# Kitware/SMQTK-Indexing

Measured on AMD Instinct MI355X. Metric: queries/sec, exact brute-force l2 kNN k=100 over 10000000x128 float32 (recall@100 = 1.0 by construction); scan HBM GB/s vs 8 TB/s peak, higher is better.
Workload: dtype f32 results (distances bit-identical to numpy float32); filter arithmetic int8 MFMA (i32 accumulation, measured per-row error bound), exact re-rank f32

## Files before the change

### smqtk_indexing_amd/csrc/sq_dense.hip

```cpp
#include <algorithm>
#include <type_traits>
#include <vector>
#include <cmath>

#include "sq_dense_exact.hpp"
#include "sq_dense_scan.hpp"
#include "sq_dense_mid.hpp"
#include "sq_dense_i8.hpp"
#include "sq_dense_wide.hpp"
#include "sq_dense_i8_wide.hpp"
#include "sq_dense_tighten.hpp"
#include "sq_dense_remove.hpp"

namespace sq {

struct DenseCall {
    bool pending = false;
    const float* q = nullptr;
    int nq = 0, k = 0, nq_pad = 0;
    void* out_dist = nullptr;
    long long* out_idx = nullptr;
    hipStream_t st = nullptr;
    bool small = false, all_fallback = false, prof = false, use_event = false, int8 = false;
    bool mid_direct = false;
// ... 560 lines not shown
            hipGraph_t g = nullptr;
            bool ok = hipStreamBeginCapture(st, hipStreamCaptureModeThreadLocal) == hipSuccess;
            if (ok) {
                const int rc = chain(st, static_cast<const DenseCallPtrs*>(ind_dev));
                const hipError_t ec = hipStreamEndCapture(st, &g);
                ok = rc == SQ_OK && ec == hipSuccess && g != nullptr;
            }
            if (ok) ok = hipGraphInstantiate(&s.gexec, g, nullptr, nullptr, 0) == hipSuccess;
            if (g) (void)hipGraphDestroy(g);
            if (!ok) {
                (void)hipGetLastError();
                s.gexec = nullptr;
                h->graph_broken = true;
            } else {
                s.gkey = key;
                if (getenv("SQ_INT8_REPORT")) fprintf(stderr, "[smqtk_hip] call graph captured (%d queries, k = %d)\n", c.nq, c.k);
            }
        }
        s.seen_key = key;
        if (s.gexec) {
            *static_cast<DenseCallPtrs*>(s.call_ptrs.p) = DenseCallPtrs{c.q, c.out_dist, c.out_idx};
            SQ_HIP(hipGraphLaunch(s.gexec, st));
            return SQ_OK;
        }
    }
    return chain(st, nullptr);
}

static int dense8_enqueue(DenseHandle* h, DenseSlot& s, const DenseCtx& e) {
    const long long n = h->n;
    DenseCall& c = s.call;
    const int d = h->d;
    c.int8 = true;
    dense8_rearm(h);
    const int row8 = h->row8, unit_rows = i8_unit_rows(row8), spu = 2 * (unit_rows / 32), waves8 = i8_waves(row8);
    const long long n_units = (n + unit_rows - 1) / unit_rows;
    long long stride = h->opt.sample_stride;
    if (stride <= 0) {
        stride = (long long)((row8 == 128 ? 14.0 : 10.0) * sqrt((double)n / 1e7 * 100.0 / (double)e.kk / (double)e.qt) / (e.cosine ? 1.9 : 1.0) + 0.5);
        if (stride > 16) stride = 16;
        const bool will_tighten = h->opt.dense_fused != 0 && h->opt.dense_tighten != 0 && e.qt == 1 && e.nqt == 1;
        if (will_tighten) {
            stride = (long long)(40.0 * sqrt((double)n / 1e7 * 100.0 / (double)e.kk) + 0.5);
            if (stride > 64) stride = 64;
        }
        if (stride < 1) stride = 1;
        if (stride > (long long)e.cap / (16ll * e.kk)) stride = std::max<long long>(1, (long long)e.cap / (16ll * e.kk));
    }
    while (stride > 1 && (n_units / stride) * spu < 8ll * e.kk) stride >>= 1;
    const long long ns_units = (n_units + stride - 1) / stride;
    const long long ns = ns_units * spu;
    SQ_TRY(s.keys.reserve((size_t)c.nq * e.key_stride * e.key_bytes));
    SQ_TRY(s.q8.reserve((size_t)2 * c.nq_pad * row8));
    SQ_TRY(s.par8.reserve((size_t)c.nq_pad * 8));
    const int cus = cu_count(h->device);
    int nrb_sample = 0;
    const int nrb = dense_pass_blocks(h->opt, c.use_event, e.nqt, cus, 0, nrb_sample);
    const long long n_waves = (long long)nrb * e.nqt * waves8;
    const int ldq = (d + 3) / 4 * 4;
    SQ_TRY(s.wave_out.reserve((size_t)n_waves * kWaveCap * 8));
    SQ_TRY(s.wave_cnt.reserve((size_t)n_waves * 8));
    SQ_TRY(s.q_al.reserve((size_t)c.nq * ldq * 4));
    const float* centerp = (!e.cosine && h->center.p) ? h->center.as<float>() : nullptr;
    Dense8ScanArgs a{};
    a.scan8 = h->scan8.as<signed char>();
    a.nrow = h->nrow8.as<float>();
    a.n = n;
    a.n_units = n_units;
    a.qs8 = s.q8.as<signed char>();
    a.par = s.par8.as<float2>();
    a.thr = e.thr;
    a.wave_out = s.wave_out.as<uint2>();
    a.wave_cnt = s.wave_cnt.as<u32>();
    a.wave_cap = kWaveCap;
    a.sample_out = s.sample.as<float>();
    a.ns = ns;
    a.nqt = e.nqt;
    a.plane_rows = c.nq_pad;
    a.debug = h->opt.dense_debug;
    dense_nt_policy(h->opt, (size_t)h->n_pad64 * row8, row8, 64, e.nqt == 1, a.nt, a.nt_from_row);
    if (ns_units < (long long)nrb_sample * waves8) nrb_sample = (int)(((ns_units + waves8 - 1) / waves8 + 7) / 8 * 8);
    bool fused = h->opt.dense_fused != 0 && e.qt == 1 && e.nqt == 1 && ns_units >= 2ll * e.kk;
    const bool tighten = fused && h->opt.dense_tighten != 0;
    if (fused) {
        const int lanes_per_wg = waves8 * 2;
        const int wg_min = ((4 * e.kk + lanes_per_wg - 1) / lanes_per_wg + 7) / 8 * 8, wg_max = 2048 / lanes_per_wg;
        if (wg_min > wg_max || wg_min > cus)
            fused = false;
        else
            nrb_sample = std::min(std::max(nrb_sample, wg_min), std::min(wg_max, (cus + 7) / 8 * 8));
    }
    int keep8 = waves8 * 2;
    if (fused) {
        const double per_wg = (double)e.kk / nrb_sample;
        if (per_wg <= 1.7 && keep8 > 4) keep8 = 4;
        else if (per_wg <= 4.5 && keep8 > 8) keep8 = 8;
    }
    const long long lane_m = (long long)nrb_sample * keep8;
    SQ_TRY(s.sample.reserve(fused ? (size_t)TILE_ROWS * lane_m * 4 : (size_t)c.nq_pad * ns * 4));
    a.sample_out = s.sample.as<float>();
    if (fused) {
        SQ_TRY(s.wave_score.reserve((size_t)n_waves * kWaveCap * 4));
        SQ_TRY(s.hist8.reserve((size_t)I8_HIST_WORDS * 4));
        a.wave_score = s.wave_score.as<float>();
        a.hist = s.hist8.as<u32>();
    }
    int wpb = 2;
    if (!e.cosine && h->opt.dense_rerank_segments > 0 && waves8 % h->opt.dense_rerank_segments == 0 && h->opt.dense_rerank_segments <= 4)
        wpb = h->opt.dense_rerank_segments;
    const double* cnx = h->cos_nx.as<double>();
    auto chain = [&](hipStream_t cs, const DenseCallPtrs* ind) -> int {
        if (fused) {
            Dense8HeadArgs ha{};
            ha.s = a;
            ha.s.unit_step = stride;
            ha.s.n_sel = ns_units;
            ha.s.nrb = nrb_sample;
            ha.q = c.q;
            ha.nq = c.nq;
            ha.d = d;
            ha.center = centerp;
            ha.dx = h->dx8;
            ha.r_max = h->rmax8;
            ha.x_max = h->xmax8;
            ha.cosine = e.cosine ? 1 : 0;
            ha.qn2 = e.qn2;
            ha.cnt = e.cnt;
            ha.oflag = e.oflag;
            ha.q_al = s.q_al.as<float>();
            ha.ldq = ldq;
            ha.ind = ind;
            ha.lane_min = s.sample.as<float>();
            ha.keep = keep8;
            ha.kk = e.kk;
            SQ_TRY(dense8_head_launch(row8, ha, cs));
            Dense8ScanArgs b = a;
            b.unit_step = 1;
            b.n_sel = n_units;
            b.nrb = nrb;
            Dense8TailArgs ta{h->db, h->ld, d, s.q_al.as<float>(), ldq, c.nq, s.keys.p, e.cnt, e.cap, e.oflag, cnx, e.cnq, h->opt.dense_debug, e.qn2, e.kk,
                              tighten ? 1 : 0, nullptr};
            s.clk8_wgs = 0;
            if ((h->opt.dense_debug & 8192) && !c.use_event) {
                SQ_TRY(s.clk8.reserve((size_t)nrb * 64));
                SQ_HIP(hipMemsetAsync(s.clk8.p, 0, (size_t)nrb * 64, cs));
                ta.clk = s.clk8.as<long long>();
                s.clk8_wgs = nrb;
            }
            if (c.prof) SQ_HIP(hipEventRecord(s.ev[1], cs));
            SQ_TRY(dense8_body_launch(row8, e.cosine, b, ta, cs));
            if (c.prof) {
                SQ_HIP(hipEventRecord(s.ev[2], cs));
                SQ_HIP(hipEventRecord(s.ev[4], cs));
            }
            return by_metric(e.cosine, [&](auto m) {
                using M = decltype(m);
                using K = typename M::Key;
                auto fin = e.filter_fin<M>();
                fin.lin = s.par8.as<float2>();
                fin.ind = ind;
                if (tighten) fin.thr2k = a.hist + TILE_ROWS * I8_HIST_BINS;
                fin.cnt_shift = I8_CNT_SHIFT;
                return select_launch_t<K>(s.keys.as<K>(), e.cnt, e.cap, e.key_stride, c.k, c.nq, s.out_keys.as<K>(), fin, cs, s.sort_tmp, 8 * stride * e.kk,
                                          I8_CNT_SHIFT);
            });
        }
        SQ_TRY(with_row8(row8, [&](auto ks) {
            return launch<dense8_prep_queries_kernel<decltype(ks)::value / 2>>(dim3(c.nq_pad / 4), dim3(64), 0, cs, c.q, c.nq, d, centerp, h->dx8, h->rmax8,
                                                                               h->xmax8, s.q8.as<signed char>(), s.par8.as<float2>(), e.qn2, e.thr, e.cnt,
                                                                               e.oflag, s.q_al.as<float>(), ldq, ind, e.cosine ? 1 : 0, c.nq_pad);
        }));
        Dense8ScanArgs b = a;
        b.unit_step = stride;
        b.n_sel = ns_units;
        b.nrb = nrb_sample;
        SQ_TRY(dense8_scan_any<true>(row8, e.qt, b, cs));
        SQ_TRY(launch<kth_threshold_f32_kernel<Dense8ThrPost>>(dim3(c.nq), dim3(1024), 0, cs, a.sample_out, ns, e.kk, e.thr,
                                                               Dense8ThrPost{s.par8.as<float2>(), e.qn2}));
        b.unit_step = 1;
        b.n_sel = n_units;
        b.nrb = nrb;
        if (c.prof) SQ_HIP(hipEventRecord(s.ev[1], cs));
        SQ_TRY(dense8_scan_any<false>(row8, e.qt, b, cs));
        if (c.prof) SQ_HIP(hipEventRecord(s.ev[2], cs));
        DenseSurvivors v = dense_slot_survivors(h, s, n_waves, wpb, ldq);
        v.expect = 8 * stride * e.kk;
        return by_metric(e.cosine, [&](auto m) {
            using M = decltype(m);
            auto fin = e.filter_fin<M>();
            fin.lin = s.par8.as<float2>();
            fin.ind = ind;
            return dense_survivor_tail<M>(h, e, v, c.k, fin, cs);
        });
    };
    c.stats.scan_launches = 2;
    c.stats.bytes_scanned = h->n_pad64 * ((long long)row8 + 4) * e.nqt;
    return dense8_launch_chain(
        h, s,
        {(u64)(fused ? 1 : 0), (u64)(tighten ? 1 : 0), (u64)(uintptr_t)s.wave_score.p, (u64)(uintptr_t)s.hist8.p, (u64)lane_m, (u64)c.nq, (u64)c.k, (u64)row8,
         (u64)e.qt, (u64)e.nqt, (u64)wpb, (u64)stride, (u64)nrb, (u64)nrb_sample, (u64)ns, (u64)a.nt, (u64)a.nt_from_row, (u64)n, (u64)h->n_live, (u64)e.cap,
         (u64)h->opt.dense_debug, (u64)h->id_base, (u64)(uintptr_t)c.st, (u64)(uintptr_t)h->db, (u64)(uintptr_t)centerp, (u64)(uintptr_t)h->scan8.p,
         (u64)(uintptr_t)h->nrow8.p, (u64)(uintptr_t)s.q8.p, (u64)(uintptr_t)s.par8.p, (u64)(uintptr_t)s.sample.p, (u64)(uintptr_t)s.keys.p,
         (u64)(uintptr_t)s.wave_out.p, (u64)(uintptr_t)s.wave_cnt.p, (u64)(uintptr_t)s.q_al.p, (u64)(uintptr_t)e.cnt, (u64)(uintptr_t)e.thr,
         (u64)(uintptr_t)e.qn2, (u64)(uintptr_t)e.oflag, (u64)(uintptr_t)s.out_keys.p, (u64)(uintptr_t)e.hs_cnt_dev, (u64)(uintptr_t)cnx,
         (u64)(uintptr_t)e.cnq, (u64)(e.cosine ? 1 : 0)},
        chain);
}

static int dense_bf16_enqueue(DenseHandle* h, DenseSlot& s, const DenseCtx& e) {
    const long long n = h->n;
    DenseCall& c = s.call;
    const int d = h->d, d_pad = h->d_pad;
    hipStream_t st = c.st;
    uint4* qs = s.q_scaled.as<uint4>();
    const double eps_a = (e.qp == 2 ? kEpsA2 : kEpsA1) * (e.cosine ? 0.5 : 1.0);
    const double eps_b = dense_eps_b(d_pad);
    const long long n_tiles = (n + TILE_ROWS - 1) / TILE_ROWS;
    const long long stride = dense_tile_stride(h->opt, n, n_tiles, e.kk, e.qt, e.cosine, e.cap);
    const long long ns_tiles = (n_tiles + stride - 1) / stride;
    const bool sample_runs = e.qt == 4 && e.qp == 1 && d_pad == KT;
    const long long ns = (sample_runs ? (ns_tiles + 3) / 4 * 4 : ns_tiles) * 2;
    SQ_TRY(s.sample.reserve((size_t)c.nq_pad * ns * 4));
    SQ_TRY(s.keys.reserve((size_t)c.nq * e.key_stride * e.key_bytes));
    const int cus = cu_count(h->device);
    int nrb_sample = 0;
    const int nrb = dense_pass_blocks(h->opt, c.use_event, e.nqt, cus, d_pad <= RING_MAX_DPAD ? 0 : e.qt == 1 ? 2 * cus : cus, nrb_sample);
    const int wv = d_pad > RING_MAX_DPAD ? WIDE_WAVES : scan_geometry(h->opt, d_pad, e.qt, e.qp).waves;
    const long long n_waves = (long long)nrb * e.nqt * wv;
    const int ldq = (d + 3) / 4 * 4;
    SQ_TRY(s.wave_out.reserve((size_t)n_waves * kWaveCap * 8));
    SQ_TRY(s.wave_cnt.reserve((size_t)n_waves * 8));
    SQ_TRY(s.q_al.reserve((size_t)c.nq * ldq * 4));
    const bool wide_tighten = h->opt.dense_tighten != 0 && d_pad > RING_MAX_DPAD && e.group_q <= TG_MAX_GROUP && c.nq_pad <= TG_CAP_Q;
    DenseTighten tg;
    if (wide_tighten) SQ_TRY(dense_tighten_scratch(s, (size_t)n_waves * kWaveCap, st, tg));
    const bool fused_prep = !e.cosine && e.qt == 1 && e.qp == 2 && h->opt.dense_fused_prep != 0 && d_pad <= RING_MAX_DPAD;
    const float* centerp = h->center.p ? h->center.as<float>() : nullptr;
    if (!fused_prep)
        SQ_TRY(launch<dense_prep_queries_kernel>(dim3(c.nq_pad), dim3(256), 0, st, c.q, c.nq, d, d_pad, h->metric, qs, e.qn2, e.thr, e.cnt, e.oflag,
                                                 s.q_al.as<float>(), ldq, centerp));
    DenseScanArgs a{};
    if (fused_prep) {
        a.raw_q = c.q;
        a.raw_nq = c.nq;
        a.raw_d = d;
        a.center = centerp;
    }
    a.scan = h->scan.as<uint4>();
    a.norms = e.cosine ? nullptr : (e.qp == 1 ? h->norms1.as<float>() : h->norms.as<float>());
    a.norm_step = 1;
    dense_nt_policy(h->opt, (size_t)h->n_pad * d_pad * 2, (long long)d_pad * 2, 192, true, a.nt, a.nt_from_row);
    if (e.cosine && (e.qt > 1 || e.qp == 1)) {
        a.norms = h->zeros.as<float>();
        a.norm_step = 0;
    }
    a.n = n;
    a.n_tiles = n_tiles;
    a.qs = qs;
    a.thr = e.thr;
    a.wave_out = s.wave_out.as<uint2>();
    a.wave_cnt = s.wave_cnt.as<u32>();
    a.wave_cap = kWaveCap;
    a.sample_out = s.sample.as<float>();
    a.ns = ns;
    a.nqt = e.nqt;
    a.debug = h->opt.dense_debug;
    a.tile_step = stride;
    a.n_sel = ns_tiles;
    a.nrb = nrb_sample;
    {
        const long long work = sample_runs ? (ns_tiles + 3) / 4 : ns_tiles;
        if (work < (long long)nrb * wv) a.nrb = (int)(((work + wv - 1) / wv + 7) / 8 * 8);
    }
    SQ_TRY(scan_launch<true>(h->opt, a, d_pad, e.qt, e.qp, st));
    DenseThrPost tp{e.qn2, e.cosine ? 1 : 0, filter_bound(e.cosine ? 1 : 0, eps_a, eps_b, h->xn2_max)};
    tp.traw_out = tg.traw;
    if (fused_prep) {
        tp.raw_q = c.q;
        tp.nq = c.nq;
        tp.nq_pad = c.nq_pad;
        tp.d = d;
        tp.ldq = ldq;
// ... 1223 lines not shown
```

### smqtk_indexing_amd/csrc/sq_dense_i8.hpp

```cpp
#pragma once
#include "sq_dense_scan.hpp"

namespace sq {

typedef int i32x4 __attribute__((ext_vector_type(4)));
typedef int i32x16 __attribute__((ext_vector_type(16)));

template <int KS>
struct I8Geom {
    static constexpr int ROW_BYTES = KS * 32;
    static constexpr int UNIT_ROWS = KS == 4 ? 64 : 32;
    static constexpr int TILES = UNIT_ROWS / 32;
    static constexpr int UNIT_BYTES = UNIT_ROWS * ROW_BYTES;
    static constexpr int SLOT_BYTES = UNIT_BYTES + 256;
    static constexpr int WAVES = KS <= 8 ? 8 : 4;
    static constexpr int NSTAGE = 2;
    static constexpr int PIECES = UNIT_BYTES / 1024;
    static constexpr int SAMPLES_PER_UNIT = 2 * TILES;
};
static constexpr int I8_MAX_ROW_BYTES = 512;
__host__ __device__ constexpr int i8_row_bytes(int d) { return d <= 128 ? 128 : (d <= 256 ? 256 : 512); }
__host__ __device__ constexpr int i8_unit_rows(int row_bytes) { return row_bytes == 128 ? 64 : 32; }

__device__ __forceinline__ float i8_element(float v, const float* __restrict__ center, int k, bool cosine, double inv_norm) {
// ... 292 lines not shown
    float ef = (float)e;
    if ((double)ef < e) ef = __uint_as_float(__float_as_uint(ef) + 1u);
    if (!ok && real) ef = __builtin_inff();
    par_out = make_float2((float)unit, real ? ef : 0.f);
    qn2_out = real ? Q : 0.0;
}

template <int EPL>
static __global__ __launch_bounds__(64) void dense8_prep_queries_kernel(const float* __restrict__ q, int nq, int d,
                                                                         const float* __restrict__ center, double dx, double r_max,
                                                                         double x_max, signed char* __restrict__ qs8,
                                                                         float2* __restrict__ par, double* __restrict__ qn2,
                                                                         float* __restrict__ thr, u32* __restrict__ cnt,
                                                                         u32* __restrict__ oflag, float* __restrict__ q_al, int ldq,
                                                                         const DenseCallPtrs* __restrict__ ind, int cosine, int plane_rows) {
    constexpr int row_bytes = EPL * 64;
    if (ind) q = ind->q;
    const int qi = blockIdx.x * 4 + (threadIdx.x >> 4), t = threadIdx.x & 15;
    if (t == 0) {
        thr[qi] = qi < nq ? -__builtin_inff() : __builtin_nanf("");
        cnt[qi] = 0u;
        if (qi == 0) *oflag = 0u;
    }
    if (qi < nq)
        for (int i = t; i < ldq; i += 16) q_al[(long long)qi * ldq + i] = i < d ? q[(long long)qi * d + i] : 0.f;
    float2 pr;
    double Q;
    dense8_prep_query_row<EPL>(q + (long long)qi * d, qi < nq, d, center, dx, r_max, x_max, cosine,
                               qs8 + (long long)qi * row_bytes, qs8 + (long long)(plane_rows + qi) * row_bytes, pr, Q);
    if (t == 0) {
        par[qi] = pr;
        qn2[qi] = Q;
    }
}

struct Dense8ThrPost {
    const float2* par;
    const double* qn2;
    __device__ __forceinline__ void prologue(int, double*) const {}
    __device__ __forceinline__ float operator()(int q, float t) const {
        if (!(t < __builtin_inff())) return t;
        if (!(par[q].y < __builtin_inff())) return __builtin_nanf("");
        const double tt = (double)t + 2.0 * (double)par[q].y + 4e-6 * fabs((double)t + qn2[q]);
        float r = (float)tt;
        if ((double)r < tt) r = __uint_as_float(__float_as_uint(r) + (r >= 0.f ? 1 : -1));
        return r;
    }
};

struct Dense8ScanArgs {
    const signed char* scan8;
    const float* nrow;
    long long n;
    long long n_units;
    const signed char* qs8;
    const float2* par;
    const float* thr;
    uint2* wave_out;
    u32* wave_cnt;
    u32 wave_cap;
    float* sample_out;
    long long ns;
    long long unit_step;
    long long n_sel;
    int nrb;
    int nt;
    long long nt_from_row;
    int nqt;
    int plane_rows;
    int debug;
    float* wave_score;
    u32* hist;
};

template <int KS>
__device__ __forceinline__ int i8_swz(int c, int r) {
    if constexpr (KS == 4) return c ^ ((r >> 1) & 7);
    return (c & ~15) | ((c & 15) ^ (r & 15));
}

enum { I8_EMIT = 0, I8_SAMPLE = 1, I8_LANEMIN = 2, I8_EMIT_H = 3 };

static constexpr int I8_HIST_BINS = 64;
static constexpr int I8_CNT_SHIFT = 5;
static constexpr int I8_HIST_WORDS = TILE_ROWS * I8_HIST_BINS + (TILE_ROWS << I8_CNT_SHIFT);

template <int WAVES>
__device__ __forceinline__ void dense8_hist_flush(u32* lds_hist, u32* __restrict__ ghist) {
    constexpr int PER = TILE_ROWS * I8_HIST_BINS / WAVES;
    const int lane = threadIdx.x & 63;
    const int wave = __builtin_amdgcn_readfirstlane(threadIdx.x >> 6);
#pragma unroll
    for (int i = 0; i < PER / 64; ++i) {
        const int b = wave * PER + i * 64 + lane;
        const u32 v = __hip_atomic_exchange(lds_hist + b, 0u, __ATOMIC_RELAXED, __HIP_MEMORY_SCOPE_WORKGROUP);
        if (v) __hip_atomic_fetch_add(ghist + b, v, __ATOMIC_RELAXED, __HIP_MEMORY_SCOPE_AGENT);
    }
}

template <int KS, int MODE>
__device__ __forceinline__ void dense8_stream(const Dense8ScanArgs& a, unsigned char* smem, const i32x4 (&bq)[KS], const i32x4 (&bl)[KS],
                                              float unit_lo, float thr_l, u32& wcount, float& smin, u32* lds_ticket,
                                              float inv_w_l = 0.f, u32* lds_hist = nullptr) {
    using G = I8Geom<KS>;
    constexpr bool SAMPLE = MODE == I8_SAMPLE || MODE == I8_LANEMIN;
    const int lane = threadIdx.x & 63;
    const int wave = __builtin_amdgcn_readfirstlane(threadIdx.x >> 6);
    const int r31 = lane & 31, h = lane >> 5;
    const u32 lds_base = (u32)(uintptr_t)smem;
    const u32 ring_base = lds_base + (u32)wave * (G::NSTAGE * G::SLOT_BYTES);
    const unsigned char* ring_ptr = smem + wave * (G::NSTAGE * G::SLOT_BYTES);
    const long long wave_id = (long long)blockIdx.x * G::WAVES + wave;
    const long long nwaves = (long long)a.nrb * G::WAVES;
    uint2* wout = a.wave_out + wave_id * a.wave_cap;
    float* wsc = MODE == I8_EMIT_H ? a.wave_score + wave_id * a.wave_cap : nullptr;
    u32* hist_l = MODE == I8_EMIT_H ? lds_hist + r31 * I8_HIST_BINS : nullptr;

    const long long wg_first = (long long)blockIdx.x * G::WAVES;
    auto take_unit = [&]() __attribute__((always_inline)) -> long long {
        u32 t = 0;
        if (lane == 0) t = __hip_atomic_fetch_add(lds_ticket, 1u, __ATOMIC_RELAXED, __HIP_MEMORY_SCOPE_WORKGROUP);
        t = (u32)__builtin_amdgcn_readfirstlane((int)t);
        const long long u = wg_first + (long long)(t % G::WAVES) + (long long)(t / G::WAVES) * nwaves;
        return u < a.n_sel ? u : -1ll;
    };
    const long long my_units = wave_id < a.n_sel ? (a.n_sel - wave_id + nwaves - 1) / nwaves : 0;
    u32 voff[G::PIECES];
#pragma unroll
    for (int j = 0; j < G::PIECES; ++j) {
        const int lin = j * 1024 + lane * 16;
        const int r = lin / G::ROW_BYTES, cpos = (lin % G::ROW_BYTES) >> 4;
        voff[j] = (u32)(r * G::ROW_BYTES + i8_swz<KS>(cpos, r) * 16);
    }
    const u32 voff_n = (u32)lane * 4u;
    static_assert(G::NSTAGE == 2, "two ring slots: the units in flight are sel_even / sel_odd");
    long long issued = 0, sel_even = -1, sel_odd = -1;
    bool more = true;
    auto issue_next = [&]() __attribute__((always_inline)) {
        if (!more) return;
        const long long sel = take_unit();
        if (sel < 0) {
            more = false;
            return;
        }
        if (issued & 1) sel_odd = sel; else sel_even = sel;
        const long long unit_idx = sel * a.unit_step;
        const long long row0 = unit_idx * G::UNIT_ROWS;
        const u32 dst = ring_base + (u32)(issued % G::NSTAGE) * G::SLOT_BYTES;
        const unsigned char* base = reinterpret_cast<const unsigned char*>(a.scan8) + row0 * G::ROW_BYTES;
#pragma unroll
        for (int j = 0; j < G::PIECES; ++j) {
            if (a.nt && row0 >= a.nt_from_row)
                glds16<true>(base, voff[j], dst + (u32)j * 1024);
            else
                glds16<false>(base, voff[j], dst + (u32)j * 1024);
        }
        glds4(a.nrow + row0, voff_n, dst + G::UNIT_BYTES);
        ++issued;
    };
    for (int p = 0; p < G::NSTAGE; ++p) issue_next();
    const int flush_every = (int)(my_units >> 3) > 0 ? (int)(my_units >> 3) : 1;
    int to_flush = flush_every;

    for (long long it = 0; it < issued; ++it) {
        const long long sel = (it & 1) ? sel_odd : sel_even;
        const long long unit_idx = sel * a.unit_step;
        const long long row0 = unit_idx * G::UNIT_ROWS;
        wait_units_in_flight<G::NSTAGE, G::PIECES + 1>((int)(issued - it - 1));
        const unsigned char* sl = ring_ptr + (it % G::NSTAGE) * G::SLOT_BYTES;
        constexpr int KH = KS == 16 ? 8 : KS;
        i32x4 av[G::TILES][KH];
        f32x4 nr[G::TILES][4];
#pragma unroll
        for (int t = 0; t < G::TILES; ++t) {
            const int r = 32 * t + r31;
#pragma unroll
            for (int s = 0; s < KH; ++s)
                av[t][s] = *reinterpret_cast<const i32x4*>(sl + r * G::ROW_BYTES + i8_swz<KS>(2 * s + h, r) * 16);
#pragma unroll
            for (int c = 0; c < 4; ++c) nr[t][c] = *reinterpret_cast<const f32x4*>(sl + G::UNIT_BYTES + (32 * t + 8 * c + 4 * h) * 4);
        }
        asm volatile("s_waitcnt lgkmcnt(0)" ::: "memory");
        if constexpr (KS != 16) issue_next();
#pragma unroll
        for (int t = 0; t < G::TILES; ++t) {
            i32x16 acc, acl;
#pragma unroll
            for (int i = 0; i < 16; ++i) acc[i] = acl[i] = 0;
#pragma unroll
            for (int s = 0; s < KH; ++s) {
                acc = __builtin_amdgcn_mfma_i32_32x32x32_i8(av[t][s], bq[s], acc, 0, 0, 0);
                acl = __builtin_amdgcn_mfma_i32_32x32x32_i8(av[t][s], bl[s], acl, 0, 0, 0);
            }
            if constexpr (KS == 16) {
#pragma unroll
                for (int s = 0; s < KH; ++s)
                    av[t][s] = *reinterpret_cast<const i32x4*>(sl + r31 * G::ROW_BYTES + i8_swz<KS>(2 * (KH + s) + h, r31) * 16);
                asm volatile("s_waitcnt lgkmcnt(0)" ::: "memory");
                issue_next();
#pragma unroll
                for (int s = 0; s < KH; ++s) {
                    acc = __builtin_amdgcn_mfma_i32_32x32x32_i8(av[t][s], bq[KH + s], acc, 0, 0, 0);
                    acl = __builtin_amdgcn_mfma_i32_32x32x32_i8(av[t][s], bl[KH + s], acl, 0, 0, 0);
                }
            }
            if (a.debug & 1024) {
                if (acc[0] == 0x7fffffff && acl[5] == 0x7ffffffe) wcount += 1;
                continue;
            }
            float sc[16];
#pragma unroll
            for (int i = 0; i < 16; ++i) {
                float nv = nr[t][i >> 2][i & 3];
                if constexpr (SAMPLE) nv = nv == -__builtin_inff() ? __builtin_inff() : nv;
                sc[i] = __fmaf_rn((float)((acc[i] << 8) + acl[i]), unit_lo, nv);
            }
            float m = sc[0];
#pragma unroll
            for (int i = 1; i < 16; ++i) m = fminf(m, sc[i]);
            if constexpr (MODE == I8_LANEMIN) {
                smin = fminf(smin, m);
            } else if constexpr (MODE == I8_SAMPLE) {
                a.sample_out[(long long)r31 * a.ns + sel * G::SAMPLES_PER_UNIT + t * 2 + h] = m;
            } else {
                const u64 hit = __ballot(m <= thr_l);
                if (hit != 0) {
                    u32 mask = 0;
#pragma unroll
                    for (int i = 0; i < 16; ++i) mask |= (sc[i] <= thr_l ? 1u : 0u) << i;
                    const u64 bal = __ballot(mask != 0);
                    if (mask) {
                        const u32 pos = wcount + __builtin_amdgcn_mbcnt_hi((u32)(bal >> 32), __builtin_amdgcn_mbcnt_lo((u32)bal, 0u));
                        if (pos < a.wave_cap) {
                            wout[pos] = make_uint2((u32)(row0 + 32 * t + 4 * h), (mask << 16) | (u32)r31);
                            if constexpr (MODE == I8_EMIT_H) wsc[pos] = m;
                        }
                        if constexpr (MODE == I8_EMIT_H) {
                            if (m > -__builtin_inff()) {
                                const int bin = min((int)((thr_l - m) * inv_w_l), I8_HIST_BINS - 1);
                                __hip_atomic_fetch_add(hist_l + bin, 1u, __ATOMIC_RELAXED, __HIP_MEMORY_SCOPE_WORKGROUP);
                            }
                        }
                    }
                    wcount += (u32)__popcll(bal);
                }
            }
        }
        if constexpr (MODE == I8_EMIT_H) {
            if (--to_flush == 0) {
                to_flush = flush_every;
                dense8_hist_flush<G::WAVES>(lds_hist, a.hist);
            }
        }
    }
}

template <int KS>
__device__ __forceinline__ void dense8_load_planes(const signed char* planes, i32x4 (&bq)[KS], i32x4 (&bl)[KS]) {
    using G = I8Geom<KS>;
    const int lane = threadIdx.x & 63, r31 = lane & 31, h = lane >> 5;
#pragma unroll
    for (int s = 0; s < KS; ++s) {
        bq[s] = *reinterpret_cast<const i32x4*>(planes + r31 * G::ROW_BYTES + (2 * s + h) * 16);
        bl[s] = *reinterpret_cast<const i32x4*>(planes + (TILE_ROWS + r31) * G::ROW_BYTES + (2 * s + h) * 16);
    }
#pragma unroll
    for (int s = 0; s < KS; ++s) asm volatile("" : "+v"(bq[s]), "+v"(bl[s]));
}

template <int KS, bool SAMPLE>
__global__ __launch_bounds__(I8Geom<KS>::WAVES * 64, KS == 16 ? 1 : 2) void dense8_scan_kernel(Dense8ScanArgs a) {
    using G = I8Geom<KS>;
    extern __shared__ __attribute__((aligned(16))) unsigned char smem[];
    const int lane = threadIdx.x & 63;
    const int wave = __builtin_amdgcn_readfirstlane(threadIdx.x >> 6);
    const int r31 = lane & 31;
    i32x4 bq[KS], bl[KS];
    dense8_load_planes<KS>(a.qs8, bq, bl);
    float unit_lo = a.par[r31].x * 0.00390625f;
    float thr_l = SAMPLE ? 0.f : a.thr[r31];
    asm volatile("" : "+v"(unit_lo), "+v"(thr_l));
    u32 wcount = 0;
    float smin = 0.f;
    __shared__ u32 s_unit_ticket;
    if (threadIdx.x == 0) s_unit_ticket = 0u;
    __syncthreads();
    dense8_stream<KS, SAMPLE ? I8_SAMPLE : I8_EMIT>(a, smem, bq, bl, unit_lo, thr_l, wcount, smin, &s_unit_ticket);
    if constexpr (!SAMPLE) {
        if (lane == 0) {
            const long long wave_id = (long long)blockIdx.x * G::WAVES + wave;
            a.wave_cnt[2 * wave_id] = wcount;
            a.wave_cnt[2 * wave_id + 1] = 0u;
        }
    }
}


struct Dense8HeadArgs {
    Dense8ScanArgs s;
    const float* q;
    int nq, d;
    const float* center;
    double dx, r_max, x_max;
    int cosine;
    double* qn2;
    u32* cnt;
    u32* oflag;
    float* q_al;
    int ldq;
    const DenseCallPtrs* ind;
    float* lane_min;
    int keep;
    int kk;
};

template <int VM, int NQ>
__device__ __forceinline__ void wave_kth_smallest(const float* __restrict__ vals, long long stride, int M, int k, float (&out)[NQ]) {
    const int lane = threadIdx.x & 63;
    constexpr u32 KINF = 0xff800000u;
    u32 key[NQ][VM];
    u32 prefix[NQ];
    u32 xall = 0u;
#pragma unroll
    for (int n = 0; n < NQ; ++n) {
        u32 kmin = KINF, kmax = 0u;
#pragma unroll
        for (int j = 0; j < VM; ++j) {
            const int i = j * 64 + lane;
            u32 kv = ordered_f32(vals[n * stride + (i < M ? i : 0)]);
            kv = (i < M && kv < KINF) ? kv : KINF;
            key[n][j] = kv;
            kmin = kv < kmin ? kv : kmin;
            kmax = kv > kmax ? kv : kmax;
        }
// ... 103 lines not shown
            for (int j = kk2 >> 1; j > 0; j >>= 1) {
                const float o = __shfl_xor(v, j);
                const bool up = (l16 & kk2) == 0, lower = (l16 & j) == 0;
                v = (lower == up) ? fminf(v, o) : fmaxf(v, o);
            }
        if (l16 < keep) ha.lane_min[(long long)qi * M + (long long)blockIdx.x * keep + l16] = v;
    }
    asm volatile("s_waitcnt vmcnt(0)" ::: "memory");
    __syncthreads();
    if (threadIdx.x == 0) {
        __threadfence();
        const u32 t = atomicAdd(&ha.oflag[1], 1u);
        if (t == gridDim.x - 1) {
            __threadfence();
            ha.oflag[1] = 0u;
        }
        s_ticket = t;
    }
    __syncthreads();
    if (s_ticket != gridDim.x - 1) return;
    float* thr = const_cast<float*>(a.thr);
    const Dense8ThrPost post{s_par, s_qn2};
#pragma unroll
    for (int rnd = 0; rnd < TILE_ROWS / (4 * G::WAVES); ++rnd) {
        const int q0 = rnd * 4 * G::WAVES + wave * 4;
        float ts[4] = {-__builtin_inff(), -__builtin_inff(), -__builtin_inff(), -__builtin_inff()};
        if (q0 < ha.nq && !(a.debug & 2048)) {
            const float* v = ha.lane_min + (long long)q0 * M;
            if (M <= 256)
                wave_kth_smallest<4, 4>(v, M, M, ha.kk, ts);
            else if (M <= 512)
                wave_kth_smallest<8, 4>(v, M, M, ha.kk, ts);
            else if (M <= 1024)
                wave_kth_smallest<16, 4>(v, M, M, ha.kk, ts);
            else {
#pragma unroll
                for (int j = 0; j < 4; ++j) {
                    float one[1];
                    wave_kth_smallest<32, 1>(v + (long long)j * M, M, M, ha.kk, one);
                    ts[j] = one[0];
                }
            }
        }
#pragma unroll
        for (int j = 0; j < 4; ++j) {
            const float t = q0 + j < ha.nq ? post(q0 + j, ts[j]) : __builtin_nanf("");
            if (lane == 0) thr[q0 + j] = t;
        }
    }
}

struct Dense8TailArgs {
    const float* db;
    long long ld;
    int d;
    const float* q_al;
    int ldq, nq;
    void* keys;
    u32* cnt;
    u32 cap;
    u32* overflow;
    const double* nx64;
    const double* nq64;
    int debug;
    const double* qn2;
    int kk;
    int tighten;
    long long* clk;
};
static constexpr int I8_TAIL_QROWS_BYTES = 32 * (156 + 4) * 4;
static constexpr int I8_TAIL_LIST = 2048;
static constexpr int I8_TAIL_RERANK_BYTES = I8_TAIL_QROWS_BYTES + 3 * RERANK_MAX_GROUP * 4 + 8 * 32 * RERANK_STAGE_STRIDE * 4;
static constexpr int I8_TAIL_LDS_BYTES = I8_TAIL_RERANK_BYTES + I8_TAIL_LIST * 8 + TILE_ROWS * 4 + 16;

template <int KS, bool COSINE>
__global__ __launch_bounds__(I8Geom<KS>::WAVES * 64, KS == 16 ? 1 : 2) void dense8_body_kernel(Dense8ScanArgs a, Dense8TailArgs ta) {
    using G = I8Geom<KS>;
    static_assert(I8_TAIL_LDS_BYTES <= G::WAVES * G::NSTAGE * G::SLOT_BYTES, "the re-rank works in the ring's LDS");
    extern __shared__ __attribute__((aligned(16))) unsigned char smem[];
    __shared__ u32 s_hist8[TILE_ROWS * I8_HIST_BINS];
    __shared__ u32 s_wcnt[G::WAVES];
    __shared__ u32 s_unit_ticket;
    __shared__ float s_thr1[TILE_ROWS], s_eq[TILE_ROWS];
    __shared__ double s_qn2b[TILE_ROWS];
    __shared__ float2 s_parb[TILE_ROWS];
    if (threadIdx.x == 0) s_unit_ticket = 0u;
    if (threadIdx.x < TILE_ROWS) {
        s_thr1[threadIdx.x] = a.thr[threadIdx.x];
        s_parb[threadIdx.x] = a.par[threadIdx.x];
        s_eq[threadIdx.x] = a.par[threadIdx.x].y;
        s_qn2b[threadIdx.x] = ta.qn2[threadIdx.x];
    }
    const int lane = threadIdx.x & 63;
    const int wave = __builtin_amdgcn_readfirstlane(threadIdx.x >> 6);
    const int r31 = lane & 31;
    for (int i = threadIdx.x; i < TILE_ROWS * I8_HIST_BINS; i += G::WAVES * 64) s_hist8[i] = 0u;
    long long* clk = ta.clk ? ta.clk + (long long)blockIdx.x * 8 : nullptr;
    if (clk && threadIdx.x == 0) {
        clk[0] = (long long)wall_clock64();
        clk[1] = 0x7fffffffffffffffll;
    }
    __syncthreads();
    i32x4 bq[KS], bl[KS];
    dense8_load_planes<KS>(a.qs8, bq, bl);
    float unit_lo = a.par[r31].x * 0.00390625f;
    float thr_l = a.thr[r31];
    const float eq_l = a.par[r31].y;
    float inv_w_l = (eq_l > 0.f && eq_l < __builtin_inff()) ? 2.f / eq_l : 0.f;
    if (!(inv_w_l < 3.0e38f)) inv_w_l = 0.f;
    asm volatile("" : "+v"(unit_lo), "+v"(thr_l), "+v"(inv_w_l));
    u32 wcount = 0;
    float smin = 0.f;
    dense8_stream<KS, I8_EMIT_H>(a, smem, bq, bl, unit_lo, thr_l, wcount, smin, &s_unit_ticket, inv_w_l, s_hist8);
    const long long w0 = (long long)blockIdx.x * G::WAVES;
    if (lane == 0) {
        a.wave_cnt[2 * (w0 + wave)] = wcount;
        a.wave_cnt[2 * (w0 + wave) + 1] = 0u;
        s_wcnt[wave] = wcount;
        if (clk) atomicMin((unsigned long long*)(clk + 1), (unsigned long long)wall_clock64());
    }
    asm volatile("s_waitcnt vmcnt(0) lgkmcnt(0)" ::: "memory");
    __builtin_amdgcn_fence(__ATOMIC_RELEASE, "workgroup");
    __syncthreads();
    __builtin_amdgcn_fence(__ATOMIC_ACQUIRE, "workgroup");
    if (clk && threadIdx.x == 0) clk[2] = (long long)wall_clock64();
    float* fl = reinterpret_cast<float*>(smem);
    u32* su = reinterpret_cast<u32*>(smem + I8_TAIL_QROWS_BYTES);
    RerankLds L{fl, su, su + RERANK_MAX_GROUP, su + 2 * RERANK_MAX_GROUP,
                COSINE ? reinterpret_cast<float*>(smem + I8_TAIL_QROWS_BYTES + 3 * RERANK_MAX_GROUP * 4) : nullptr};
    {
        uint2* s_list = reinterpret_cast<uint2*>(smem + I8_TAIL_RERANK_BYTES);
        float* s_thr2 = reinterpret_cast<float*>(smem + I8_TAIL_RERANK_BYTES + I8_TAIL_LIST * 8);
        u32* s_npass = reinterpret_cast<u32*>(s_thr2 + TILE_ROWS);
        static_assert(I8_HIST_BINS == 64, "one lane per bin");
        bool any = false;
#pragma unroll
        for (int wi = 0; wi < G::WAVES; ++wi) any = any || s_wcnt[wi] != 0u;
        const Dense8ThrPost post{s_parb, s_qn2b};
        constexpr int NQW = TILE_ROWS / G::WAVES;
        u32 hc[NQW];
        if (ta.tighten && any) {
#pragma unroll
            for (int j = 0; j < NQW; ++j) {
                const int qi = (j >> 2) * 4 * G::WAVES + wave * 4 + (j & 3);
                hc[j] = __hip_atomic_load(a.hist + qi * I8_HIST_BINS + lane, __ATOMIC_RELAXED, __HIP_MEMORY_SCOPE_AGENT);
            }
#pragma unroll
            for (int j = 0; j < NQW; ++j) {
                const int qi = (j >> 2) * 4 * G::WAVES + wave * 4 + (j & 3);
                hc[j] += s_hist8[qi * I8_HIST_BINS + lane];
            }
        }
#pragma unroll
        for (int rnd = 0; rnd < TILE_ROWS / (4 * G::WAVES); ++rnd) {
#pragma unroll
            for (int j = 0; j < 4; ++j) {
                const int qi = rnd * 4 * G::WAVES + wave * 4 + j;
                const float t1 = s_thr1[qi];
                float t2 = t1;
                if (ta.tighten && any && qi < ta.nq && t1 < __builtin_inff() && t1 > -__builtin_inff()) {
                    u32 c = hc[rnd * 4 + j];
#pragma unroll
                    for (int o = 1; o < 64; o <<= 1) {
                        const u32 up = (u32)__shfl_down((int)c, o);
                        c += lane + o < 64 ? up : 0u;
                    }
                    const u64 reach = __ballot(c >= (u32)ta.kk);
                    const float eq = s_eq[qi];
                    if (reach != 0ull && eq > 0.f && eq < __builtin_inff()) {
                        const int jb = 63 - __clzll((long long)reach);
                        const float inv_w = 2.f / eq;
                        if (inv_w < 3.0e38f) {
                            const double t8 = (double)t1 - (double)jb / (double)inv_w * (1.0 - 1e-6);
                            float t8f = (float)t8;
                            if ((double)t8f < t8) t8f = __uint_as_float(__float_as_uint(t8f) + (t8f >= 0.f ? 1 : -1));
                            const float cand = post(qi, t8f);
                            if (cand < t2) t2 = cand;
                        }
                    }
                    if (lane == 0) atomicMax(a.hist + TILE_ROWS * I8_HIST_BINS + (qi << I8_CNT_SHIFT), ordered_f32(t2));
                }
                if (lane == 0) s_thr2[qi] = t2;
            }
        }
        if (ta.tighten) {
            L.scores = a.wave_score;
            L.thr2 = s_thr2;
            L.list = s_list;
            L.npass = s_npass;
            L.list_cap = I8_TAIL_LIST;
        }
        L.seg_cnt = s_wcnt;
        L.cnt_shift = I8_CNT_SHIFT;
        __syncthreads();
        if (clk && threadIdx.x == 0) clk[3] = (long long)wall_clock64();
        if (ta.tighten) dense8_hist_flush<G::WAVES>(s_hist8, a.hist);
    }
    using K = typename std::conditional<COSINE, K128, u64>::type;
    rerank_block<K, COSINE>(ta.db, ta.ld, ta.d, ta.q_al, ta.ldq, ta.nq, TILE_ROWS, a.wave_out, a.wave_cnt, a.wave_cap,
                            (long long)a.nrb * G::WAVES, G::WAVES, static_cast<K*>(ta.keys), ta.cnt, ta.cap, ta.overflow, ta.nx64,
                            ta.nq64, ta.debug, w0, L);
    if (clk) {
        asm volatile("s_waitcnt vmcnt(0) lgkmcnt(0)" ::: "memory");
        __syncthreads();
        if (threadIdx.x == 0) clk[4] = (long long)wall_clock64();
    }
}

template <int QT, bool SAMPLE>
__global__ __launch_bounds__(512, 2) void dense8_scan_mt_kernel(Dense8ScanArgs a) {
    using G = I8Geom<4>;
    extern __shared__ __attribute__((aligned(16))) unsigned char smem[];
    const int lane = threadIdx.x & 63;
    const int wave = __builtin_amdgcn_readfirstlane(threadIdx.x >> 6);
    const int r31 = lane & 31, h = lane >> 5;
    const u32 lds_base = (u32)(uintptr_t)smem;
    const u32 ring_base = lds_base + (u32)wave * (G::NSTAGE * G::SLOT_BYTES);
    const unsigned char* ring_ptr = smem + wave * (G::NSTAGE * G::SLOT_BYTES);
    const long long wave_id = (long long)blockIdx.x * G::WAVES + wave;
    uint2* wout = a.wave_out + wave_id * a.wave_cap;
    const int L = blockIdx.x;
    int grp, rb;
    if (a.nqt > 1) {
        const int xcd = L & 7, j = L >> 3;
        grp = j % a.nqt;
        rb = (j / a.nqt) * 8 + xcd;
    } else {
        grp = 0;
        rb = L;
    }
    const int q_first = grp * QT * TILE_ROWS;
    const long long rwave = (long long)rb * G::WAVES + wave, nwaves = (long long)a.nrb * G::WAVES;

    i32x4 bq[QT][4], bl[QT][4];
    float unit_lo[QT], thr_l[QT];
#pragma unroll
    for (int g = 0; g < QT; ++g) {
        const int qg = q_first + g * TILE_ROWS + r31;
#pragma unroll
        for (int s = 0; s < 4; ++s) {
            bq[g][s] = *reinterpret_cast<const i32x4*>(a.qs8 + (long long)qg * G::ROW_BYTES + (2 * s + h) * 16);
            bl[g][s] = *reinterpret_cast<const i32x4*>(a.qs8 + (long long)(a.plane_rows + qg) * G::ROW_BYTES + (2 * s + h) * 16);
        }
        unit_lo[g] = a.par[qg].x * 0.00390625f;
        thr_l[g] = SAMPLE ? 0.f : a.thr[qg];
        asm volatile("" : "+v"(unit_lo[g]), "+v"(thr_l[g]));
#pragma unroll
        for (int s = 0; s < 4; ++s) asm volatile("" : "+v"(bq[g][s]), "+v"(bl[g][s]));
    }

    const long long my_units = rwave < a.n_sel ? (a.n_sel - rwave + nwaves - 1) / nwaves : 0;
    u32 voff[G::PIECES];
#pragma unroll
    for (int j = 0; j < G::PIECES; ++j) {
        const int r = 8 * j + (lane >> 3);
        voff[j] = (u32)(r * G::ROW_BYTES + i8_swz<4>(lane & 7, r) * 16);
    }
    const u32 voff_n = (u32)lane * 4u;
    long long issued = 0;
    auto issue_next = [&]() __attribute__((always_inline)) {
        if (issued >= my_units) return;
        const long long unit_idx = (rwave + issued * nwaves) * a.unit_step;
// ... 82 lines not shown
```

Before: 149,400.

## Refresh int8 filter threshold mid-scan from global histogram

Adds scheduled in-stream refreshes: at a few points during the fused int8 scan, one wave per workgroup reads the global and local histograms, computes a tightened per-query threshold via a DPP prefix sum, and publishes it to shared memory with a CAS-min. The scan loop then loads the current threshold each unit, so fewer candidates are emitted and fewer survivors reach the exact f32 re-rank. The tighten option gains modes 2 and 3 that control whether refresh and tail histogram tightening run. The cost is extra atomic loads, histogram reads and per-unit LDS loads inside the hot loop, plus stalls for the wave doing the refresh.

```diff
diff --git a/smqtk_indexing_amd/csrc/sq_dense.hip b/smqtk_indexing_amd/csrc/sq_dense.hip
--- a/smqtk_indexing_amd/csrc/sq_dense.hip
+++ b/smqtk_indexing_amd/csrc/sq_dense.hip
@@ -666,6 +666,7 @@
     if (ns_units < (long long)nrb_sample * waves8) nrb_sample = (int)(((ns_units + waves8 - 1) / waves8 + 7) / 8 * 8);
     bool fused = h->opt.dense_fused != 0 && e.qt == 1 && e.nqt == 1 && ns_units >= 2ll * e.kk;
     const bool tighten = fused && h->opt.dense_tighten != 0;
+    const int tighten_mode = !tighten ? 0 : (h->opt.dense_tighten == 2 || h->opt.dense_tighten == 3) ? h->opt.dense_tighten : 1;
     if (fused) {
         const int lanes_per_wg = waves8 * 2;
         const int wg_min = ((4 * e.kk + lanes_per_wg - 1) / lanes_per_wg + 7) / 8 * 8, wg_max = 2048 / lanes_per_wg;
@@ -723,7 +724,7 @@
             b.n_sel = n_units;
             b.nrb = nrb;
             Dense8TailArgs ta{h->db, h->ld, d, s.q_al.as<float>(), ldq, c.nq, s.keys.p, e.cnt, e.cap, e.oflag, cnx, e.cnq, h->opt.dense_debug, e.qn2, e.kk,
-                              tighten ? 1 : 0, nullptr};
+                              tighten_mode, nullptr};
             s.clk8_wgs = 0;
             if ((h->opt.dense_debug & 8192) && !c.use_event) {
                 SQ_TRY(s.clk8.reserve((size_t)nrb * 64));
@@ -781,7 +782,7 @@
     c.stats.bytes_scanned = h->n_pad64 * ((long long)row8 + 4) * e.nqt;
     return dense8_launch_chain(
         h, s,
-        {(u64)(fused ? 1 : 0), (u64)(tighten ? 1 : 0), (u64)(uintptr_t)s.wave_score.p, (u64)(uintptr_t)s.hist8.p, (u64)lane_m, (u64)c.nq, (u64)c.k, (u64)row8,
+        {(u64)(fused ? 1 : 0), (u64)tighten_mode, (u64)(uintptr_t)s.wave_score.p, (u64)(uintptr_t)s.hist8.p, (u64)lane_m, (u64)c.nq, (u64)c.k, (u64)row8,
          (u64)e.qt, (u64)e.nqt, (u64)wpb, (u64)stride, (u64)nrb, (u64)nrb_sample, (u64)ns, (u64)a.nt, (u64)a.nt_from_row, (u64)n, (u64)h->n_live, (u64)e.cap,
          (u64)h->opt.dense_debug, (u64)h->id_base, (u64)(uintptr_t)c.st, (u64)(uintptr_t)h->db, (u64)(uintptr_t)centerp, (u64)(uintptr_t)h->scan8.p,
          (u64)(uintptr_t)h->nrow8.p, (u64)(uintptr_t)s.q8.p, (u64)(uintptr_t)s.par8.p, (u64)(uintptr_t)s.sample.p, (u64)(uintptr_t)s.keys.p,
diff --git a/smqtk_indexing_amd/csrc/sq_dense_i8.hpp b/smqtk_indexing_amd/csrc/sq_dense_i8.hpp
--- a/smqtk_indexing_amd/csrc/sq_dense_i8.hpp
+++ b/smqtk_indexing_amd/csrc/sq_dense_i8.hpp
@@ -398,6 +398,9 @@
 enum { I8_EMIT = 0, I8_SAMPLE = 1, I8_LANEMIN = 2, I8_EMIT_H = 3 };
 
 static constexpr int I8_HIST_BINS = 64;
+static constexpr int I8_EVENTS = 7, I8_REFRESHES = 4;
+static constexpr int I8_SCHED_MIN_UNITS = 32;
+__device__ __forceinline__ int i8_event_at(int units, int e) { return (units * (e < 4 ? (1 << e) : 2 * e + 2)) >> 4; }
 static constexpr int I8_CNT_SHIFT = 5;
 static constexpr int I8_HIST_WORDS = TILE_ROWS * I8_HIST_BINS + (TILE_ROWS << I8_CNT_SHIFT);
 
@@ -414,10 +417,92 @@
     }
 }
 
+__device__ __forceinline__ float dense8_thr_from_bin(int jb, float t1, float eq, int qi, const Dense8ThrPost& post) {
+    float t2 = t1;
+    if (jb >= 0 && eq > 0.f && eq < __builtin_inff()) {
+        const float inv_w = 2.f / eq;
+        if (inv_w < 3.0e38f) {
+            const double t8 = (double)t1 - (double)jb / (double)inv_w * (1.0 - 1e-6);
+            float t8f = (float)t8;
+            if ((double)t8f < t8) t8f = __uint_as_float(__float_as_uint(t8f) + (t8f >= 0.f ? 1 : -1));
+            const float cand = post(qi, t8f);
+            if (cand < t2) t2 = cand;
+        }
+    }
+    return t2;
+}
+
+__device__ __forceinline__ float dense8_tightened(u32 c, float t1, float eq, int kk, int qi, const Dense8ThrPost& post) {
+    static_assert(I8_HIST_BINS == 64, "one lane per bin");
+    const int lane = threadIdx.x & 63;
+#pragma unroll
+    for (int o = 1; o < 64; o <<= 1) {
+        const u32 up = (u32)__shfl_down((int)c, o);
+        c += lane + o < 64 ? up : 0u;
+    }
+    const u64 reach = __ballot(c >= (u32)kk);
+    const int jb = reach != 0ull ? 63 - __clzll((long long)reach) : -1;
+    return dense8_thr_from_bin(jb, t1, eq, qi, post);
+}
+
+struct Dense8StreamTighten {
+    u32* hist;
+    float* thr_cur;
+    const float* thr1;
+    const float* eq;
+    Dense8ThrPost post;
+    int kk, nq;
+    int refresh;
+};
+
+__device__ __forceinline__ u32 wave_prefix_sum_dpp(u32 v) {
+    v += (u32)__builtin_amdgcn_update_dpp(0, (int)v, 0x111, 0xf, 0xf, false);
+    v += (u32)__builtin_amdgcn_update_dpp(0, (int)v, 0x112, 0xf, 0xf, false);
+    v += (u32)__builtin_amdgcn_update_dpp(0, (int)v, 0x114, 0xf, 0xf, false);
+    v += (u32)__builtin_amdgcn_update_dpp(0, (int)v, 0x118, 0xf, 0xf, false);
+    v += (u32)__builtin_amdgcn_update_dpp(0, (int)v, 0x142, 0xa, 0xf, false);
+    v += (u32)__builtin_amdgcn_update_dpp(0, (int)v, 0x143, 0xc, 0xf, false);
+    return v;
+}
+
+__device__ __forceinline__ void dense8_refresh(const Dense8StreamTighten& tg, const u32* __restrict__ ghist) {
+    const int lane = threadIdx.x & 63;
+    constexpr int NB = 16;
+    int jb_l = -1;
+#pragma unroll 1
+    for (int q0 = 0; q0 < TILE_ROWS; q0 += NB) {
+        u32 hc[NB];
+#pragma unroll
+        for (int j = 0; j < NB; ++j) hc[j] = __hip_atomic_load(ghist + (q0 + j) * I8_HIST_BINS + 63 - lane, __ATOMIC_RELAXED, __HIP_MEMORY_SCOPE_AGENT);
+        asm volatile("s_waitcnt vmcnt(0)" ::: "memory");
+#pragma unroll
+        for (int j = 0; j < NB; ++j) asm volatile("" : "+v"(hc[j]));
+#pragma unroll
+        for (int j = 0; j < NB; ++j) hc[j] += __hip_atomic_load(tg.hist + (q0 + j) * I8_HIST_BINS + 63 - lane, __ATOMIC_RELAXED, __HIP_MEMORY_SCOPE_WORKGROUP);
+#pragma unroll
+        for (int j = 0; j < NB; ++j) {
+            const u64 reach = __ballot(wave_prefix_sum_dpp(hc[j]) >= (u32)tg.kk);
+            const int jb = reach != 0ull ? 63 - (int)__builtin_ctzll(reach) : -1;
+            jb_l = lane == q0 + j ? jb : jb_l;
+        }
+    }
+    const float t1 = tg.thr1[lane & 31];
+    if (lane < TILE_ROWS && lane < tg.nq && t1 < __builtin_inff() && t1 > -__builtin_inff()) {
+        const float t2 = dense8_thr_from_bin(jb_l, t1, tg.eq[lane], lane, tg.post);
+        u32* p = reinterpret_cast<u32*>(tg.thr_cur + lane);
+        u32 old = __hip_atomic_load(p, __ATOMIC_RELAXED, __HIP_MEMORY_SCOPE_WORKGROUP);
+        while (t2 < __uint_as_float(old)) {
+            const u32 seen = atomicCAS(p, old, __float_as_uint(t2));
+            if (seen == old) break;
+            old = seen;
+        }
+    }
+}
+
 template <int KS, int MODE>
 __device__ __forceinline__ void dense8_stream(const Dense8ScanArgs& a, unsigned char* smem, const i32x4 (&bq)[KS], const i32x4 (&bl)[KS],
                                               float unit_lo, float thr_l, u32& wcount, float& smin, u32* lds_ticket,
-                                              float inv_w_l = 0.f, u32* lds_hist = nullptr) {
+                                              float inv_w_l = 0.f, const Dense8StreamTighten* tg = nullptr) {
     using G = I8Geom<KS>;
     constexpr bool SAMPLE = MODE == I8_SAMPLE || MODE == I8_LANEMIN;
     const int lane = threadIdx.x & 63;
@@ -430,7 +515,10 @@
     const long long nwaves = (long long)a.nrb * G::WAVES;
     uint2* wout = a.wave_out + wave_id * a.wave_cap;
     float* wsc = MODE == I8_EMIT_H ? a.wave_score + wave_id * a.wave_cap : nullptr;
+    u32* lds_hist = nullptr;
+    if constexpr (MODE == I8_EMIT_H) lds_hist = tg->hist;
     u32* hist_l = MODE == I8_EMIT_H ? lds_hist + r31 * I8_HIST_BINS : nullptr;
+    float thr_c = thr_l;
 
     const long long wg_first = (long long)blockIdx.x * G::WAVES;
     auto take_unit = [&]() __attribute__((always_inline)) -> long long {
@@ -477,6 +565,12 @@
     for (int p = 0; p < G::NSTAGE; ++p) issue_next();
     const int flush_every = (int)(my_units >> 3) > 0 ? (int)(my_units >> 3) : 1;
     int to_flush = flush_every;
+    bool sched = false, refresh_next = false;
+    int ev = 0, ev_gap = 0;
+    if constexpr (MODE == I8_EMIT_H) {
+        sched = tg->refresh != 0 && my_units >= I8_SCHED_MIN_UNITS && my_units < (1ll << 24);
+        if (sched) to_flush = i8_event_at((int)my_units, 0);
+    }
 
     for (long long it = 0; it < issued; ++it) {
         const long long sel = (it & 1) ? sel_odd : sel_even;
@@ -496,7 +590,10 @@
 #pragma unroll
             for (int c = 0; c < 4; ++c) nr[t][c] = *reinterpret_cast<const f32x4*>(sl + G::UNIT_BYTES + (32 * t + 8 * c + 4 * h) * 4);
         }
+        float thr_n = thr_c;
+        if constexpr (MODE == I8_EMIT_H) thr_n = __hip_atomic_load(tg->thr_cur + r31, __ATOMIC_RELAXED, __HIP_MEMORY_SCOPE_WORKGROUP);
         asm volatile("s_waitcnt lgkmcnt(0)" ::: "memory");
+        if constexpr (MODE == I8_EMIT_H) thr_c = thr_n < thr_c ? thr_n : thr_c;
         if constexpr (KS != 16) issue_next();
 #pragma unroll
         for (int t = 0; t < G::TILES; ++t) {
@@ -539,11 +636,11 @@
             } else if constexpr (MODE == I8_SAMPLE) {
                 a.sample_out[(long long)r31 * a.ns + sel * G::SAMPLES_PER_UNIT + t * 2 + h] = m;
             } else {
-                const u64 hit = __ballot(m <= thr_l);
+                const u64 hit = __ballot(m <= thr_c);
                 if (hit != 0) {
                     u32 mask = 0;
 #pragma unroll
-                    for (int i = 0; i < 16; ++i) mask |= (sc[i] <= thr_l ? 1u : 0u) << i;
+                    for (int i = 0; i < 16; ++i) mask |= (sc[i] <= thr_c ? 1u : 0u) << i;
                     const u64 bal = __ballot(mask != 0);
                     if (mask) {
                         const u32 pos = wcount + __builtin_amdgcn_mbcnt_hi((u32)(bal >> 32), __builtin_amdgcn_mbcnt_lo((u32)bal, 0u));
@@ -564,8 +661,24 @@
         }
         if constexpr (MODE == I8_EMIT_H) {
             if (--to_flush == 0) {
-                to_flush = flush_every;
                 dense8_hist_flush<G::WAVES>(lds_hist, a.hist);
+                if (!sched) {
+                    to_flush = flush_every;
+                } else if (refresh_next) {
+                    refresh_next = false;
+                    dense8_refresh(*tg, a.hist);
+                    to_flush = ev_gap - 1;
+                } else {
+                    const int gap = ev + 1 < I8_EVENTS ? i8_event_at((int)my_units, ev + 1) - i8_event_at((int)my_units, ev) : 0x7fffffff;
+                    if (ev < I8_REFRESHES && wave == ev % G::WAVES) {
+                        refresh_next = true;
+                        ev_gap = gap;
+                        to_flush = 1;
+                    } else {
+                        to_flush = gap;
+                    }
+                    ++ev;
+                }
             }
         }
     }
@@ -835,11 +948,13 @@
     __shared__ u32 s_wcnt[G::WAVES];
     __shared__ u32 s_unit_ticket;
     __shared__ float s_thr1[TILE_ROWS], s_eq[TILE_ROWS];
+    __shared__ float s_thrc[TILE_ROWS];
     __shared__ double s_qn2b[TILE_ROWS];
     __shared__ float2 s_parb[TILE_ROWS];
     if (threadIdx.x == 0) s_unit_ticket = 0u;
     if (threadIdx.x < TILE_ROWS) {
         s_thr1[threadIdx.x] = a.thr[threadIdx.x];
+        s_thrc[threadIdx.x] = a.thr[threadIdx.x];
         s_parb[threadIdx.x] = a.par[threadIdx.x];
         s_eq[threadIdx.x] = a.par[threadIdx.x].y;
         s_qn2b[threadIdx.x] = ta.qn2[threadIdx.x];
@@ -864,7 +979,8 @@
     asm volatile("" : "+v"(unit_lo), "+v"(thr_l), "+v"(inv_w_l));
     u32 wcount = 0;
     float smin = 0.f;
-    dense8_stream<KS, I8_EMIT_H>(a, smem, bq, bl, unit_lo, thr_l, wcount, smin, &s_unit_ticket, inv_w_l, s_hist8);
+    const Dense8StreamTighten tg{s_hist8, s_thrc, s_thr1, s_eq, Dense8ThrPost{s_parb, s_qn2b}, ta.kk, ta.nq, (ta.tighten == 1 || ta.tighten == 3) ? 1 : 0};
+    dense8_stream<KS, I8_EMIT_H>(a, smem, bq, bl, unit_lo, thr_l, wcount, smin, &s_unit_ticket, inv_w_l, &tg);
     const long long w0 = (long long)blockIdx.x * G::WAVES;
     if (lane == 0) {
         a.wave_cnt[2 * (w0 + wave)] = wcount;
@@ -885,14 +1001,14 @@
         uint2* s_list = reinterpret_cast<uint2*>(smem + I8_TAIL_RERANK_BYTES);
         float* s_thr2 = reinterpret_cast<float*>(smem + I8_TAIL_RERANK_BYTES + I8_TAIL_LIST * 8);
         u32* s_npass = reinterpret_cast<u32*>(s_thr2 + TILE_ROWS);
-        static_assert(I8_HIST_BINS == 64, "one lane per bin");
         bool any = false;
 #pragma unroll
         for (int wi = 0; wi < G::WAVES; ++wi) any = any || s_wcnt[wi] != 0u;
         const Dense8ThrPost post{s_parb, s_qn2b};
         constexpr int NQW = TILE_ROWS / G::WAVES;
         u32 hc[NQW];
-        if (ta.tighten && any) {
+        const bool from_hist = ta.tighten == 1 || ta.tighten == 2;
+        if (from_hist && any) {
 #pragma unroll
             for (int j = 0; j < NQW; ++j) {
                 const int qi = (j >> 2) * 4 * G::WAVES + wave * 4 + (j & 3);
@@ -912,25 +1028,7 @@
                 const float t1 = s_thr1[qi];
                 float t2 = t1;
                 if (ta.tighten && any && qi < ta.nq && t1 < __builtin_inff() && t1 > -__builtin_inff()) {
-                    u32 c = hc[rnd * 4 + j];
-#pragma unroll
-                    for (int o = 1; o < 64; o <<= 1) {
-                        const u32 up = (u32)__shfl_down((int)c, o);
-                        c += lane + o < 64 ? up : 0u;
-                    }
-                    const u64 reach = __ballot(c >= (u32)ta.kk);
-                    const float eq = s_eq[qi];
-                    if (reach != 0ull && eq > 0.f && eq < __builtin_inff()) {
-                        const int jb = 63 - __clzll((long long)reach);
-                        const float inv_w = 2.f / eq;
-                        if (inv_w < 3.0e38f) {
-                            const double t8 = (double)t1 - (double)jb / (double)inv_w * (1.0 - 1e-6);
-                            float t8f = (float)t8;
-                            if ((double)t8f < t8) t8f = __uint_as_float(__float_as_uint(t8f) + (t8f >= 0.f ? 1 : -1));
-                            const float cand = post(qi, t8f);
-                            if (cand < t2) t2 = cand;
-                        }
-                    }
+                    t2 = from_hist ? dense8_tightened(hc[rnd * 4 + j], t1, s_eq[qi], ta.kk, qi, post) : s_thrc[qi];
                     if (lane == 0) atomicMax(a.hist + TILE_ROWS * I8_HIST_BINS + (qi << I8_CNT_SHIFT), ordered_f32(t2));
                 }
                 if (lane == 0) s_thr2[qi] = t2;
```

Result: slower. 146,400 (-2.0%).
